# X1X1010/XequiNet

Hardware: AMD Instinct MI355X
Metric: edges/sec + achieved HBM GB/s, energy+force inference, QM9-shape batch (higher is better)
Workload: dtype f32

## Files before the change

include/xeq.h:

```cpp
#ifndef XEQ_H
#define XEQ_H
#include <stdint.h>

#ifdef __cplusplus
extern "C" {
#endif

enum { XEQ_F32 = 0, XEQ_F64 = 1 };
enum { XEQ_RBF_BESSEL = 0, XEQ_RBF_GAUSSIAN = 1, XEQ_RBF_EXPBERN = 2, XEQ_RBF_EXPNORM = 3 };
enum { XEQ_CUTOFF_COSINE = 0, XEQ_CUTOFF_POLYNOMIAL = 1 };
enum {
  XEQ_OK = 0,
  XEQ_ERR_INVALID_ARGUMENT = 1,
  XEQ_ERR_LAUNCH = 2,
  XEQ_ERR_UNSUPPORTED = 3
};

int xeq_version(void);
const char* xeq_last_error(void);
int64_t xeq_launch_count(void);
int64_t xeq_launch_names(int64_t first, char* buf, int64_t cap);


int xeq_csr_rowptr(const int64_t* keys, int64_t n_keys, int64_t n_rows, int32_t* rowptr, void* stream);
// ... 173 lines not shown
int xeq_message_param_grad_mc(int64_t n_nodes, int64_t n_edges, const int64_t* center, const int64_t* nbr, const void* tab, const void* h,
                              const void* xhat, const void* grad_s, const void* grad_x, int rbf_kind, int num_basis, int node_dim,
                              const int32_t mul[3], int xhat_layout, int grad_x_layout, const int32_t* n_valid, int n_parts, void* parts,
                              void* stream);
int xeq_norm_param_grad_chunks(int64_t n_nodes);
int xeq_norm_param_grad(const void* s, const void* x, const void* stats, const void* g_shat, int64_t ld_gs, const void* g_xhat_bt,
                        int64_t n_nodes, int node_dim, const int32_t mul[3], int n_chunks, void* parts, void* stream);
int xeq_to_bt(const void* x, int64_t n_nodes, const int32_t mul[3], void* out, void* stream);

int xeq_train_norm(int dtype, int reverse, int64_t n, const void* s, const void* s_tan, const void* x, const void* x_tan, const void* ln_w,
                   const void* ln_b, const void* eq_w, const void* eq_b, const void* g_s, const void* g_x, int node_dim,
                   const int32_t mul[3], double eps_ln, double eps_eq, int xhat_layout, void* out_s, void* out_x, void* rows, void* stream);
int xeq_train_uv(int dtype, int reverse, int64_t n, const void* const uv[3], const void* const uv_tan[3], const void* g, const int32_t mul[3],
                 double eps, void* out, void* const d_uv[3], void* stream);
int xeq_train_out(int dtype, int reverse, int64_t n, const void* const uv[3], const void* const uv_tan[3], const void* a, const void* a_tan,
                  const void* inner, const void* inner_tan, const void* g_s, const void* g_x, int node_dim, const int32_t mul[3],
                  void* out0, void* out1, void* const d_uv[3], void* stream);

#define XEQ_FAMILY_WQ 0
#define XEQ_FAMILY_SB 1
#define XEQ_FAMILY_GENERIC 3
int xeq_message_auto_family(int dtype, int64_t n_nodes, int64_t n_edges, int num_basis, int node_dim, const int32_t mul[3]);
int xeq_message_wq_edges_per_stream(int64_t n_nodes, int64_t n_edges);

int xeq_edge_basis_width(int num_basis);
int xeq_message_sb_fits(int64_t n_nodes, int64_t n_edges, int num_basis, int node_dim, const int32_t mul[3]);
int xeq_edge_basis(int dtype, const void* vec, int64_t n_edges, int rbf_kind, int cutoff_kind, int num_basis,
                   double cutoff, const void* p0, const void* p1, void* basis, void* dbasis, void* stream);
int xeq_message_fwd_sb(int dtype, int64_t n_nodes, int64_t n_edges, const int32_t* rowptr, const int32_t* perm,
                       const int64_t* nbr, const void* basis, const void* h, const void* xhat, const void* s_in,
                       const void* x_in, const void* w_rbf, const void* b_rbf, int num_basis, int node_dim,
                       const int32_t mul[3], void* s_out, void* x_out, int xhat_layout, void* stream);
int xeq_message_bwd_sb(int dtype, int64_t n_nodes, int64_t n_edges, const int32_t* n_rowptr, const int32_t* n_perm,
                       const int64_t* center, const void* basis, const void* dbasis, const void* h, const void* xhat,
                       const void* grad_s, const void* grad_x, const void* w_rbf, const void* b_rbf, int num_basis,
                       int node_dim, const int32_t mul[3], void* grad_h, void* grad_xhat, void* grad_vec,
                       int xhat_layout, void* stream);

#define XEQ_SB_Y0_ZERO 8
#define XEQ_SB_ACCUM_VEC 16
#define XEQ_SB_Q_ACCUMULATE 16
#define XEQ_SB_NO_GY 32
int xeq_message_bwd_sbq(int dtype, int64_t n_nodes, int64_t n_edges, const int32_t* n_rowptr, const int32_t* n_perm,
                        const int64_t* center, const void* basis, const void* h, const void* xhat, const void* grad_s,
                        const void* grad_x, const void* w_rbf, const void* b_rbf, int num_basis, int node_dim,
                        const int32_t mul[3], void* grad_h, void* grad_xhat, void* q, void* gy, int flags, void* stream);
int xeq_message_fwd_sb_pair(int dtype, int64_t n_nodes, int64_t n_edges, const int32_t* rowptr, const int32_t* perm, const int64_t* nbr,
                            const void* basis, const void* basis_u, const void* h, const void* u_h, const void* xhat, const void* u_xhat,
                            const void* s_in, const void* x_in, const void* w_rbf, const void* b_rbf, int num_basis, int node_dim,
                            const int32_t mul[3], void* s_out, void* x_out, int xhat_layout, void* stream);
int xeq_message_bwd_sbq_pair(int dtype, int64_t n_nodes, int64_t n_edges, const int32_t* n_rowptr, const int32_t* n_perm,
                             const int64_t* center, const void* basis, const void* basis_u, const void* h, const void* u_h, const void* xhat,
                             const void* u_xhat, const void* grad_s, const void* grad_x, const void* w_rbf, const void* b_rbf, int num_basis,
                             int node_dim, const int32_t mul[3], void* grad_h, void* grad_xhat, void* q, void* gy, int flags, void* stream);
int xeq_zero_rows_from(void* buf, int64_t row_words, int64_t n_rows, const int32_t* n_valid, void* stream);
int xeq_message_q_wgrad_chunks(int64_t n_edges);
int xeq_message_q_wgrad(int dtype, const void* q, const void* basis, int64_t n_edges, int num_basis, int node_dim, const int32_t mul[3],
                        int n_chunks, void* parts, void* stream);

int xeq_message_wq_supported(int num_basis, int node_dim, const int32_t mul[3]);
int xeq_message_wq_fits(int64_t n_nodes, int64_t n_edges, int num_basis, int node_dim, const int32_t mul[3]);
int64_t xeq_message_wq_pcap(int64_t n_nodes, int64_t n_edges);
int xeq_message_wq_waves(void);
int xeq_message_wq_record_floats_for(int num_basis);
int xeq_message_wq_record_floats(void);
int64_t xeq_message_wq_plan_workspace(int64_t n_nodes);
int64_t xeq_message_wq_win_ints(int n_ranges);
int xeq_message_wq_plan(const int32_t* rowptr, const int32_t* perm, const int64_t* owner, const int64_t* gather,
                        int64_t n_nodes, int64_t n_edges, int n_ranges, void* workspace, int64_t workspace_bytes,
                        int32_t* qptr, int32_t* pgath, int32_t* peid, int32_t* qinfo, int32_t* sq, int32_t* sn, int32_t* win,
                        void* stream);
int xeq_edge_basis_wq(const void* vec, int64_t n_nodes, int64_t n_edges, const int32_t* qptr, const int32_t* peid,
                      int rbf_kind, int cutoff_kind, int num_basis, double cutoff, const void* p0, const void* p1,
                      void* basis, void* dbasis, void* stream);
int xeq_message_fwd_wq(int64_t n_nodes, int64_t n_edges, int n_ranges, const int32_t* sq, const int32_t* sn, const int32_t* win,
                       const int32_t* c_rowptr, const int32_t* pgath, const int32_t* qinfo, const void* basis, const void* h,
                       const void* xhat, const void* s_in, const void* x_in, const void* w_rbf, const void* b_rbf,
                       int num_basis, int node_dim, const int32_t mul[3], void* s_out, void* x_out, int xhat_layout,
                       void* stream);
int64_t xeq_message_wq_parts_floats(int64_t n_nodes, int64_t n_edges, const int32_t mul[3]);
#define XEQ_XHAT_HIGHER_L_ZERO 2
#define XEQ_WQ_MIRROR_WALK 4
#define XEQ_WQ_PACKED_WEIGHTS 64
int64_t xeq_message_wq_packed_weight_floats(int num_basis, int node_dim, const int32_t mul[3]);
int xeq_message_wq_pack_weights(const void* w_rbf, const void* b_rbf, int num_basis, int node_dim, const int32_t mul[3], void* packed,
                                void* stream);
int xeq_message_bwd_wq(int64_t n_nodes, int64_t n_edges, int n_ranges, const int32_t* sq, const int32_t* sn, const int32_t* win,
                       const int32_t* n_rowptr, const int32_t* pgath, const int32_t* qinfo, const void* basis,
                       const void* dbasis, const void* h, const void* xhat, const void* grad_s, const void* grad_x,
                       const void* w_rbf, const void* b_rbf, int num_basis, int node_dim, const int32_t mul[3], void* grad_h,
                       void* grad_xhat, void* parts, int xhat_layout, void* stream);
int xeq_message_wq_edge_grad(const void* vec, int64_t n_nodes, int64_t n_edges, const int32_t* qptr, const int32_t* peid,
                             const int32_t* mirror, const int32_t mul[3], const void* parts, void* grad_vec, void* stream);
#define XEQ_WQ_MAX_PART_SETS 8
// ... 85 lines not shown
```

xequinet_amd/csrc/xeq_message_wq.hip:

```cpp
#include "xeq_common.h"

#include <hipcub/hipcub.hpp>
#include <stdlib.h>

namespace xeq {

typedef float f32x16 __attribute__((ext_vector_type(16)));
typedef float f32x4 __attribute__((ext_vector_type(4)));
typedef int i32x4 __attribute__((ext_vector_type(4)));

typedef __bf16 bf16x8 __attribute__((ext_vector_type(8)));

constexpr bool wq_bftail(int ks) { return ks <= 3; }
constexpr int WQ_TAIL = 24;
constexpr int wq_tailw(int ks) { return ks <= 4 ? 4 : 8; }
constexpr int wq_recf(int ks) { return WQ_TAIL + 2 * wq_tailw(ks) + 8; }
constexpr int wq_yoff(int ks) { return WQ_TAIL + 2 * wq_tailw(ks); }
constexpr int wq_tail_values(int num_basis) { return (num_basis > 16 ? num_basis - 16 : 0) + 1; }
constexpr int wq_ks(int num_basis) {
  return wq_tail_values(num_basis) <= 1 ? 1 : (wq_tail_values(num_basis) <= 5 ? 3 : ((wq_tail_values(num_basis) + 1) / 2 < 4 ? 4 : (wq_tail_values(num_basis) + 1) / 2));
}
constexpr int WQ_REC_MAX = 48;
__device__ __forceinline__ uint32_t wq_bf16_rne(float x) {
  const uint32_t u = __float_as_uint(x);
// ... 67 lines not shown
    qinfo[q0 + g] = (uint32_t)n | (g == 0 ? WQ_FIRST : 0u) | (g == nq - 1 ? WQ_LAST : 0u);
  }
}

__global__ void k_wq_streams(const int32_t* __restrict__ qptr, int64_t N, int n_ranges, int32_t* __restrict__ sq,
                             int32_t* __restrict__ sn) {
  const int k = blockIdx.x * blockDim.x + threadIdx.x;
  if (k > 2 * n_ranges) return;
  const int64_t Q = qptr[N];
  if (k == 2 * n_ranges) {
    sq[k] = (int32_t)Q;
    sn[k] = (int32_t)N;
    return;
  }
  const int64_t target = (int64_t)k * Q / (2 * n_ranges);
  int64_t lo = 0, hi = N;
  while (lo < hi) {
    const int64_t mid = (lo + hi) >> 1;
    if (qptr[mid] >= target) hi = mid;
    else lo = mid + 1;
  }
  sq[k] = qptr[lo];
  sn[k] = (int32_t)lo;
}

__global__ void k_wq_windows(const int32_t* __restrict__ sq, const int32_t* __restrict__ pgath, int n_ranges, int n_steps, int mult,
                             int32_t* __restrict__ win) {
  const int step = blockIdx.x, lane = threadIdx.x;
  if (step >= n_steps) return;
  const int k0 = min(2 * WQ_WAVES * mult * step, 2 * n_ranges), k1 = min(k0 + 2 * WQ_WAVES * mult, 2 * n_ranges);
  const int64_t p0 = 4 * (int64_t)sq[k0], p1 = 4 * (int64_t)sq[k1];
  int lo = 0x7fffffff, hi = -1;
  for (int64_t p = p0 + lane; p < p1; p += 64) {
    const int g = pgath[p];
    lo = g < lo ? g : lo;
    hi = g > hi ? g : hi;
  }
#pragma unroll
  for (int o = 32; o > 0; o >>= 1) {
    const int l2 = __shfl_xor(lo, o, 64), h2 = __shfl_xor(hi, o, 64);
    lo = l2 < lo ? l2 : lo;
    hi = h2 > hi ? h2 : hi;
  }
  if (lane == 0) {
    win[2 * step] = hi >= 0 ? lo : 0;
    win[2 * step + 1] = hi >= 0 ? hi - lo + 1 : 0;
// ... 1499 lines not shown
int xeq_message_wq_supported(int num_basis, int node_dim, const int32_t mul[3]) { return wq_supported(num_basis, node_dim, mul) ? 1 : 0; }

int xeq_message_wq_fits(int64_t n_nodes, int64_t n_edges, int num_basis, int node_dim, const int32_t mul[3]) {
  return wq_supported(num_basis, node_dim, mul) && n_nodes < (1ll << 30) && wq_fits(n_nodes, n_edges, node_dim, mul) ? 1 : 0;
}

int64_t xeq_message_wq_pcap(int64_t n_nodes, int64_t n_edges) { return wq_pcap(n_nodes, n_edges); }

int xeq_message_wq_waves(void) { return WQ_WAVES; }

int xeq_message_wq_record_floats(void) { return wq_recf(4); }
int xeq_message_wq_record_floats_for(int num_basis) { return wq_recf(wq_ks(num_basis)); }

int64_t xeq_message_wq_plan_workspace(int64_t n_nodes) {
  size_t temp = 0;
  QuadCount op{nullptr, n_nodes};
  hipcub::CountingInputIterator<int64_t> cnt(0);
  hipcub::TransformInputIterator<int32_t, QuadCount, hipcub::CountingInputIterator<int64_t>> it(cnt, op);
  if (hipcub::DeviceScan::ExclusiveSum(nullptr, temp, it, (int32_t*)nullptr, (int)(n_nodes + 1)) != hipSuccess) return -1;
  return (int64_t)temp + 256;
}

int xeq_message_wq_plan(const int32_t* rowptr, const int32_t* perm, const int64_t* owner, const int64_t* gather,
                        int64_t n_nodes, int64_t n_edges, int n_ranges, void* workspace, int64_t workspace_bytes,
                        int32_t* qptr, int32_t* pgath, int32_t* peid, int32_t* qinfo, int32_t* sq, int32_t* sn, int32_t* win,
                        void* stream) {
  XEQ_CHECK_ARG(n_nodes >= 0 && n_edges >= 0 && n_ranges >= 1 && n_nodes < (1ll << 30) && n_edges < (1ll << 31), "xeq_message_wq_plan: bad sizes");
  const int64_t need = xeq_message_wq_plan_workspace(n_nodes);
  XEQ_CHECK_ARG(need >= 0 && workspace_bytes >= need, "xeq_message_wq_plan: workspace of %lld bytes, need %lld", (long long)workspace_bytes, (long long)need);
  QuadCount op{rowptr, n_nodes};
  if (n_nodes <= SCAN_WG_MAX_ITEMS) {
    static const bool attr_ok = hipFuncSetAttribute((const void*)k_wq_quad_scan, hipFuncAttributeMaxDynamicSharedMemorySize,
                                                    (int)wg_scan_lds_bytes(SCAN_WG_MAX_ITEMS)) == hipSuccess;
    XEQ_CHECK_ARG(attr_ok, "xeq_message_wq_plan: cannot reserve LDS for the quad scan");
    hipLaunchKernelGGL(k_wq_quad_scan, dim3(1), dim3(SCAN_WG_THREADS), wg_scan_lds_bytes(n_nodes), (hipStream_t)stream, op, qptr);
    XEQ_CHECK_LAUNCH("xeq_message_wq_plan (quad scan)");
  } else {
    hipcub::CountingInputIterator<int64_t> cnt(0);
    hipcub::TransformInputIterator<int32_t, QuadCount, hipcub::CountingInputIterator<int64_t>> it(cnt, op);
    size_t temp = (size_t)workspace_bytes;
    if (hipcub::DeviceScan::ExclusiveSum(workspace, temp, it, qptr, (int)(n_nodes + 1), (hipStream_t)stream) != hipSuccess) {
      xeq::set_error("xeq_message_wq_plan: scan failed");
      return XEQ_ERR_LAUNCH;
    }
  }
  if (n_edges + n_nodes > 0) {
    hipLaunchKernelGGL(k_wq_fill, dim3((unsigned)((n_edges + n_nodes + 255) / 256)), dim3(256), 0, (hipStream_t)stream, n_edges, n_nodes,
                       rowptr, perm, owner, gather, (const int32_t*)qptr, pgath, peid, (uint32_t*)qinfo);
    XEQ_CHECK_LAUNCH("xeq_message_wq_plan (fill)");
  }
  const int n = 2 * n_ranges + 1;
  hipLaunchKernelGGL(k_wq_streams, dim3((unsigned)((n + 255) / 256)), dim3(256), 0, (hipStream_t)stream, (const int32_t*)qptr,
                     n_nodes, n_ranges, sq, sn);
  XEQ_CHECK_LAUNCH("xeq_message_wq_plan (streams)");
  const int n_steps = wq_class_steps(n_ranges, 1);
  hipLaunchKernelGGL(k_wq_windows, dim3((unsigned)n_steps), dim3(64), 0, (hipStream_t)stream, (const int32_t*)sq,
                     (const int32_t*)pgath, n_ranges, n_steps, 1, win);
  XEQ_CHECK_LAUNCH("xeq_message_wq_plan (windows)");
  const int mlong = wq_long_mult(n_edges, n_ranges);
  if (mlong > 1) {
    const int n_long = wq_class_steps(n_ranges, mlong);
    hipLaunchKernelGGL(k_wq_windows, dim3((unsigned)n_long), dim3(64), 0, (hipStream_t)stream, (const int32_t*)sq,
                       (const int32_t*)pgath, n_ranges, n_long, mlong, win + 2 * n_steps);
    XEQ_CHECK_LAUNCH("xeq_message_wq_plan (windows, long class)");
  }
  return XEQ_OK;
}

int64_t xeq_message_wq_win_ints(int n_ranges) {
  return 2 * ((int64_t)wq_class_steps(n_ranges, 1) + (int64_t)wq_class_steps(n_ranges, 2) + 1);
}

int xeq_edge_basis_wq(const void* vec, int64_t n_nodes, int64_t n_edges, const int32_t* qptr, const int32_t* peid,
                      int rbf_kind, int cutoff_kind, int num_basis, double cutoff, const void* p0, const void* p1,
                      void* basis, void* dbasis, void* stream) {
  XEQ_CHECK_ARG(n_edges >= 0 && n_nodes >= 0 && num_basis >= 1 && num_basis <= 31 && cutoff > 0, "xeq_edge_basis_wq: bad sizes");
  XEQ_CHECK_ARG(rbf_kind >= XEQ_RBF_BESSEL && rbf_kind <= XEQ_RBF_EXPNORM, "xeq_edge_basis_wq: rbf kernel %d is not implemented", rbf_kind);
  XEQ_CHECK_ARG(rbf_kind == XEQ_RBF_BESSEL || p1 != nullptr, "xeq_edge_basis_wq: this radial basis needs its second parameter array (std / logc / mu)");
  XEQ_CHECK_ARG(cutoff_kind == XEQ_CUTOFF_COSINE || cutoff_kind == XEQ_CUTOFF_POLYNOMIAL, "xeq_edge_basis_wq: cutoff function %d is not implemented", cutoff_kind);
  if (n_edges == 0 && n_nodes == 0) return XEQ_OK;
  const int64_t pcap = wq_pcap(n_nodes, n_edges), total = (pcap + WQ_REC_SLOTS - 1) / WQ_REC_SLOTS * 256;
  const int ks = wq_ks(num_basis);
  XEQ_CHECK_ARG(pcap * wq_recf(ks) < (1ll << 31) * 2, "xeq_edge_basis_wq: too many edges for 32-bit record offsets (shard the batch)");
  RadialSpec rs{rbf_kind, cutoff_kind, num_basis, cutoff};
  hipLaunchKernelGGL(k_wq_records, dim3((unsigned)((total + 255) / 256)), dim3(256), 0, (hipStream_t)stream, (const float*)vec,
                     peid, qptr, n_nodes, pcap, rs, (const float*)p0, (const float*)p1, (float*)basis, (float*)dbasis, wq_recf(ks), wq_tailw(ks), wq_bftail(ks) ? 1 : 0);
  XEQ_CHECK_LAUNCH("xeq_edge_basis_wq");
  return XEQ_OK;
}

// ... 154 lines not shown
```

xequinet_amd/csrc/xeq_ops.hip:

```cpp
#include "xeq_common.h"

namespace xeq {

template <typename T>
__global__ void k_edge_vectors_fwd(const T* __restrict__ pos, const int64_t* __restrict__ edge_index, int64_t E,
                                   const T* __restrict__ cell, const T* __restrict__ cell_offsets,
                                   const int64_t* __restrict__ batch, T* __restrict__ vec, T* __restrict__ dist) {
  int64_t e = (int64_t)blockIdx.x * blockDim.x + threadIdx.x;
  if (e >= E) return;
  int64_t c = edge_index[e], n = edge_index[E + e];
  T v[3];
#pragma unroll
  for (int a = 0; a < 3; ++a) v[a] = pos[3 * c + a] - pos[3 * n + a];
  if (cell != nullptr) {
    const T* cm = cell + (batch ? 9 * batch[n] : 0);
    T o0 = cell_offsets[3 * e], o1 = cell_offsets[3 * e + 1], o2 = cell_offsets[3 * e + 2];
#pragma unroll
    for (int a = 0; a < 3; ++a) v[a] -= o0 * cm[a] + o1 * cm[3 + a] + o2 * cm[6 + a];
  }
  vec[3 * e] = v[0];
  vec[3 * e + 1] = v[1];
  vec[3 * e + 2] = v[2];
  if (dist) dist[e] = sqrt_<T>(v[0] * v[0] + v[1] * v[1] + v[2] * v[2]);
}
// ... 303 lines not shown

__global__ void k_compare_many(CopyMany cm, int32_t gen, int32_t* __restrict__ flag) {
  const int b = blockIdx.y;
  const int64_t words = cm.bytes[b] / 4;
  const uint32_t* x = reinterpret_cast<const uint32_t*>(cm.src[b]);
  const uint32_t* y = reinterpret_cast<const uint32_t*>(cm.dst[b]);
  bool diff = false;
  for (int64_t i = (int64_t)blockIdx.x * blockDim.x + threadIdx.x; i < words; i += (int64_t)gridDim.x * blockDim.x) diff |= x[i] != y[i];
  if (__ballot(diff) != 0ull && (threadIdx.x & 63) == 0) flag[0] = gen;
}

}

using namespace xeq;

#define XEQ_IRREPS(who)                       \
  Irreps ir;                                  \
  {                                           \
    int rc_ = check_irreps(mul, ir, who);     \
    if (rc_ != XEQ_OK) return rc_;            \
  }

#include <atomic>
static std::atomic<long long> g_pack_epoch{0};

extern "C" {

long long xeq_pack_epoch(void) { return g_pack_epoch.load(); }
void xeq_pack_epoch_bump(void) { g_pack_epoch.fetch_add(1); }


int xeq_message_auto_family(int dtype, int64_t n_nodes, int64_t n_edges, int num_basis, int node_dim, const int32_t mul[3]) {
  const bool f32 = dtype == XEQ_F32;
  const bool sb_fits = xeq_message_sb_fits(n_nodes, n_edges, num_basis, node_dim, mul) != 0;
  if (n_edges < 4096 && sb_fits) return XEQ_FAMILY_SB;
  if (f32 && xeq_message_wq_fits(n_nodes, n_edges, num_basis, node_dim, mul)) return XEQ_FAMILY_WQ;
  if (sb_fits) return XEQ_FAMILY_SB;
  return XEQ_FAMILY_GENERIC;
}

int64_t xeq_small_rows_limit(void) { return xeq_small_rows(); }

int xeq_message_wq_edges_per_stream(int64_t n_nodes, int64_t n_edges) {
  const double per_node = (double)n_edges / (double)(n_nodes > 0 ? n_nodes : 1);
  double v = per_node > 16.0 ? per_node : 16.0;
  const double spread = (double)n_edges / 1500.0;
  if (spread > v) v = spread;
  if (v > 80.0) v = 80.0;
  return (int)v;
}


int xeq_edge_vectors_fwd(int dtype, const void* pos, const int64_t* edge_index, int64_t n_edges,
                         const void* cell, const void* cell_offsets, const int64_t* batch, void* vec, void* dist,
                         void* stream) {
  XEQ_CHECK_ARG(n_edges >= 0, "xeq_edge_vectors_fwd: n_edges < 0");
  XEQ_CHECK_ARG((cell == nullptr) == (cell_offsets == nullptr), "xeq_edge_vectors_fwd: cell and cell_offsets must both be given or both be NULL (data/transform.py:67-68)");
  if (n_edges == 0) return XEQ_OK;
  XEQ_DISPATCH_FLOAT(dtype, {
    hipLaunchKernelGGL((k_edge_vectors_fwd<T>), dim3((unsigned)((n_edges + 255) / 256)), dim3(256), 0,
                       (hipStream_t)stream, (const T*)pos, edge_index, n_edges, (const T*)cell,
                       (const T*)cell_offsets, batch, (T*)vec, (T*)dist);
  });
  XEQ_CHECK_LAUNCH("xeq_edge_vectors_fwd");
  return XEQ_OK;
}

int xeq_edge_vectors_bwd(int dtype, const void* grad_vec, int64_t n_nodes, const int32_t* c_rowptr,
                         const int32_t* c_perm, const int32_t* n_rowptr, const int32_t* n_perm, void* grad_pos,
                         void* stream) {
  XEQ_CHECK_ARG(n_nodes >= 0, "xeq_edge_vectors_bwd: n_nodes < 0");
  if (n_nodes == 0) return XEQ_OK;
// ... 289 lines not shown
```

xequinet_amd/csrc/xeq_torch.cpp:

```cpp
#include <ATen/ATen.h>
#include <c10/hip/HIPStream.h>
#include <hip/hip_runtime_api.h>
#include <torch/csrc/autograd/custom_function.h>
#include <torch/library.h>

#include <array>
#include <cmath>
#include <cstdlib>
#include <map>
#include <mutex>
#include <optional>
#include <unordered_map>
#include <vector>

#include "../../include/xeq.h"

namespace {

using at::Tensor;
using torch::autograd::AutogradContext;
using torch::autograd::variable_list;

#define XCALL(...)                                                                                  \
  do {                                                                                              \
// ... 225 lines not shown
struct NbPacks { Tensor fwd, bwd, bias_uv; };
const NbPacks* nb_packs(const Tensor* q, const Tensor* qn, bool gx) {
  const bool tail = qn != nullptr;
  const Tensor none;
  return &packed<NbPacks>(q[15].data_ptr(), {&q[15], &q[10], &q[11], &q[12], &q[14], &q[17], &q[13], tail ? &qn[0] : &none, tail ? &qn[2] : &none},
                          (tail ? 2 : 0) + (gx ? 1 : 0), [&](NbPacks& e) {
    const auto bopt = q[15].options().dtype(at::kByte);
    const Tensor w3 = q[15].detach().contiguous(), dot = q[14].detach().contiguous(), w4 = q[17].detach().contiguous();
    const Tensor uv0 = q[10].contiguous(), uv1 = q[11].contiguous(), uv2 = q[12].contiguous();
    Tensor w1n, w2n;
    if (tail) {
      w1n = qn[0].detach().contiguous();
      w2n = qn[2].detach().contiguous();
    }
    e.fwd = at::empty({xeq_node_block_fwd_tiles(tail) * 3072}, bopt);
    XCALL(xeq_node_block_pack_fwd(PF(w3), PF(uv0), PF(uv1), PF(uv2), PF(dot), PF(w4), PF(w1n), PF(w2n), e.fwd.data_ptr(), cur_stream()));
    e.bwd = at::empty({xeq_node_block_bwd_tiles(tail, gx) * 3072}, bopt);
    XCALL(xeq_node_block_pack_bwd(PF(w3), PF(uv0), PF(uv1), PF(uv2), PF(dot), PF(w4), PF(w1n), PF(w2n), gx, e.bwd.data_ptr(), cur_stream()));
    e.bias_uv = q[13].numel() > 0 ? q[13].detach().contiguous() : Tensor();
  });
}

struct WqPlan {
  int n_ranges = 0;
  int64_t pcap = 0;
  Tensor qptr, pgath, peid, qinfo, sq, sn, win, rowptr, work, basis, dbasis;
};
struct Graph {
  int64_t N = 0, E = 0;
  bool mirror = false;
  Tensor ei, c_rowptr, c_perm, n_rowptr, n_perm;
  Tensor mirror_map;
  WqPlan fwd, rev;
  Tensor sb_basis, sb_dbasis;
  void sorted_view();
  const Tensor& rev_rowptr() { if (!mirror_map.defined()) sorted_view(); return mirror_map.defined() ? c_rowptr : n_rowptr; }
  const Tensor& rev_perm() { if (!mirror_map.defined()) sorted_view(); return mirror_map.defined() ? mirror_map : n_perm; }
};

Tensor i32(int64_t n, const Tensor& like) { return at::empty({std::max<int64_t>(n, 1)}, like.options().dtype(at::kInt)); }

void csr_by_key(const Tensor& keys, int64_t n_rows, Tensor& rowptr, Tensor& perm) {
  const int64_t n = keys.numel(), bytes = xeq_csr_by_key_workspace(n, n_rows);
  TORCH_CHECK(bytes >= 0, "xequinet_amd: csr_by_key: sizes out of range");
  Tensor work = at::empty({std::max<int64_t>(bytes, 1)}, keys.options().dtype(at::kByte));
  rowptr = i32(n_rows + 1, keys);
  perm = i32(n, keys);
// ... 19 lines not shown
  }
  const char* env = std::getenv("XEQ_PBC_MIRROR");
  const bool periodic = cell_offsets != nullptr && cell_offsets->defined();
  g.mirror = symmetric && center_sorted && (!periodic || !(env && env[0] == '0' && env[1] == 0));
  if (g.mirror && !periodic) {
    g.n_rowptr = g.c_rowptr;
    g.n_perm = i32(g.E, g.ei);
    XCALL(xeq_reverse_edge_map((const int64_t*)g.ei.data_ptr(), g.E, n_nodes, (const int32_t*)g.c_rowptr.data_ptr(),
                               (int32_t*)g.n_perm.data_ptr(), cur_stream()));
    g.mirror_map = g.n_perm;
  } else if (g.mirror) {
    g.mirror_map = i32(g.E, g.ei);
    XCALL(xeq_reverse_edge_map_pbc(dcode(*cell_offsets), (const int64_t*)g.ei.data_ptr(), cell_offsets->data_ptr(), g.E, n_nodes,
                                   (const int32_t*)g.c_rowptr.data_ptr(), (int32_t*)g.mirror_map.data_ptr(), cur_stream()));
  } else {
    g.sorted_view();
  }
  return g;
}

void build_wq_plan(Graph& g, bool reverse, WqPlan& p) {
  if (reverse) g.sorted_view();
  const int eps = xeq_message_wq_edges_per_stream(g.N, g.E);
  p.n_ranges = (int)std::max<int64_t>(1, (g.E + 2 * eps - 1) / (2 * eps));
  p.pcap = xeq_message_wq_pcap(g.N, g.E);
  p.qptr = i32(g.N + 1, g.ei);
  p.pgath = i32(p.pcap, g.ei);
  p.peid = i32(p.pcap, g.ei);
  p.qinfo = i32(p.pcap / 4, g.ei);
  p.sq = i32(2 * p.n_ranges + 1, g.ei);
  p.sn = i32(2 * p.n_ranges + 1, g.ei);
  p.win = i32(xeq_message_wq_win_ints(p.n_ranges), g.ei);
  const int64_t wbytes = xeq_message_wq_plan_workspace(g.N);
  TORCH_CHECK(wbytes >= 0, "xequinet_amd: wq plan workspace");
  p.work = at::empty({std::max<int64_t>(wbytes, 1)}, g.ei.options().dtype(at::kByte));
  p.rowptr = reverse ? g.n_rowptr : g.c_rowptr;
  const Tensor& perm = reverse ? g.n_perm : g.c_perm;
  const Tensor owner = g.ei.select(0, reverse ? 1 : 0), gather = g.ei.select(0, reverse ? 0 : 1);
  XCALL(xeq_message_wq_plan((const int32_t*)p.rowptr.data_ptr(), perm.defined() ? (const int32_t*)perm.data_ptr() : nullptr,
                            (const int64_t*)owner.data_ptr(), (const int64_t*)gather.data_ptr(), g.N, g.E, p.n_ranges,
                            p.work.data_ptr(), wbytes, (int32_t*)p.qptr.data_ptr(), (int32_t*)p.pgath.data_ptr(),
                            (int32_t*)p.peid.data_ptr(), (int32_t*)p.qinfo.data_ptr(), (int32_t*)p.sq.data_ptr(),
                            (int32_t*)p.sn.data_ptr(), (int32_t*)p.win.data_ptr(), cur_stream()));
}

constexpr int P_BLOCK0 = 5, P_PER_BLOCK = 27, P_ELECTRONIC = 6;
struct Hyper {
  int F, mul[3], B, blocks, rbf_kind, cutoff_kind, layer_norm, embed_kind;
  double cutoff, inv_eps;
  int C() const { return mul[0] + mul[1] + mul[2]; }
  int D() const { return mul[0] + 3 * mul[1] + 5 * mul[2]; }
  int H() const { return F + 2 * C(); }
};

const Tensor* opt(const Tensor& t) { return t.defined() && t.numel() > 0 ? &t : nullptr; }
const void* OP(const Tensor& t) { return t.defined() && t.numel() > 0 ? t.data_ptr() : nullptr; }

struct BtBlock {
  int l, m;
  Tensor view;
};
std::vector<BtBlock> bt_blocks(const Tensor& buf, int64_t n, const int mul[3], int width) {
  std::vector<BtBlock> out;
  int64_t base = 0;
// ... 737 lines not shown
```

xequinet_amd/lib.py:

```python
from __future__ import annotations

import ctypes
import os
from ctypes import c_char_p, c_double, c_int, c_int32, c_int64, c_void_p
from typing import Optional

import torch

_HERE = os.path.dirname(os.path.abspath(__file__))
LIB_PATH = os.environ.get("XEQ_LIB_PATH") or os.path.join(_HERE, "libxeq_hip.so")

XEQ_F32, XEQ_F64 = 0, 1
COPY_MANY_MAX = 16
SB_ACCUM_VEC = 16
XHAT_HIGHER_L_ZERO = 2
SB_Y0_ZERO = 8
SB_Q_ACCUMULATE = 16
SB_NO_GY = 32
WQ_MIRROR_WALK = 4
WQ_PACKED_WEIGHTS = 64
WQ_MAX_PART_SETS = 8
RBF_KINDS = {"bessel": 0, "gaussian": 1, "expbern": 2, "expnorm": 3}
CUTOFF_KINDS = {"cosine": 0, "polynomial": 1}

# ... 88 lines not shown
    "xeq_edge_basis_width": [c_int],
    "xeq_edge_basis": [c_int, _P, c_int64, c_int, c_int, c_int, c_double, _P, _P, _P, _P, _P],
    "xeq_message_fwd_sb": [c_int, c_int64, c_int64, _P, _P, _P, _P, _P, _P, _P, _P, _P, _P, c_int, c_int, _I3, _P, _P, c_int, _P],
    "xeq_message_bwd_sbq": [c_int, c_int64, c_int64, _P, _P, _P, _P, _P, _P, _P, _P, _P, _P, c_int, c_int, _I3, _P, _P, _P, _P, c_int, _P],
    "xeq_message_q_wgrad": [c_int, _P, _P, c_int64, c_int, c_int, _I3, c_int, _P, _P],
    "xeq_message_q_wgrad_chunks": [c_int64],
    "xeq_train_norm": [c_int, c_int, c_int64, _P, _P, _P, _P, _P, _P, _P, _P, _P, _P, c_int, _I3, c_double, c_double, c_int, _P, _P, _P, _P],
    "xeq_train_uv": [c_int, c_int, c_int64, _P, _P, _P, _I3, c_double, _P, _P, _P],
    "xeq_train_out": [c_int, c_int, c_int64, _P, _P, _P, _P, _P, _P, _P, _P, c_int, _I3, _P, _P, _P, _P],
    "xeq_zero_rows_from": [_P, c_int64, c_int64, _P, _P],
    "xeq_message_fwd_sb_pair": [c_int, c_int64, c_int64, _P, _P, _P, _P, _P, _P, _P, _P, _P, _P, _P, _P, _P, c_int, c_int, _I3, _P, _P, c_int, _P],
    "xeq_message_bwd_sbq_pair": [c_int, c_int64, c_int64, _P, _P, _P, _P, _P, _P, _P, _P, _P, _P, _P, _P, _P, c_int, c_int, _I3, _P, _P, _P, _P, c_int, _P],
    "xeq_message_bwd_sb": [c_int, c_int64, c_int64, _P, _P, _P, _P, _P, _P, _P, _P, _P, _P, _P, c_int, c_int, _I3, _P, _P, _P,
                           c_int, _P],
    "xeq_message_sb_fits": [c_int64, c_int64, c_int, c_int, _I3],
    "xeq_message_wq_supported": [c_int, c_int, _I3],
    "xeq_message_wq_fits": [c_int64, c_int64, c_int, c_int, _I3],
    "xeq_message_wq_pcap": [c_int64, c_int64],
    "xeq_message_wq_waves": [],
    "xeq_message_wq_record_floats": [],
    "xeq_message_wq_record_floats_for": [c_int],
    "xeq_message_wq_plan_workspace": [c_int64],
    "xeq_message_wq_win_ints": [c_int],
    "xeq_message_wq_plan": [_P, _P, _P, _P, c_int64, c_int64, c_int, _P, c_int64, _P, _P, _P, _P, _P, _P, _P, _P],
    "xeq_edge_basis_wq": [_P, c_int64, c_int64, _P, _P, c_int, c_int, c_int, c_double, _P, _P, _P, _P, _P],
    "xeq_message_fwd_wq": [c_int64, c_int64, c_int, _P, _P, _P, _P, _P, _P, _P, _P, _P, _P, _P, _P, _P, c_int, c_int, _I3,
                           _P, _P, c_int, _P],
    "xeq_message_wq_parts_floats": [c_int64, c_int64, _I3],
    "xeq_message_bwd_wq": [c_int64, c_int64, c_int, _P, _P, _P, _P, _P, _P, _P, _P, _P, _P, _P, _P, _P, _P, c_int, c_int,
                           _I3, _P, _P, _P, c_int, _P],
    "xeq_message_wq_packed_weight_floats": [c_int, c_int, _I3],
    "xeq_message_wq_pack_weights": [_P, _P, c_int, c_int, _I3, _P, _P],
    "xeq_message_wq_edge_grad": [_P, c_int64, c_int64, _P, _P, _P, _I3, _P, _P, _P],
    "xeq_message_wq_edge_grad_sum": [_P, c_int64, c_int64, _P, _P, _P, _I3, c_int, ctypes.POINTER(c_void_p), _P, _P],
    "xeq_norm_fwd": [c_int, _P, _P, _P, _P, _P, _P, c_int64, c_int, _I3, c_int, _P, c_int64, _P, _P, _P],
    "xeq_norm_bwd": [c_int, _P, _P, _P, _P, _P, c_int64, c_int, _I3, c_int, _P, c_int64, _P, _P, _P, _P, _P, _P],
    "xeq_uv_reduce_fwd": [c_int, _P, c_int64, _I3, c_double, _P, c_int64, c_int, _P, _P],
    "xeq_uv_reduce_bwd": [c_int, _P, _P, _P, c_int64, c_int, c_int64, _I3, c_double, _P, _P, _P, _P],
    "xeq_update_out_fwd": [c_int, _P, _P, _P, _P, _P, c_int64, c_int, _I3, _P, _P, _P],
    "xeq_update_out_bwd": [c_int, _P, _P, _P, _P, _P, c_int64, c_int, _I3, _P, _P, _P, _P],
    "xeq_update_uv_supported": [c_int, c_int, _I3],
    "xeq_update_uv_fwd": [_P, _P, _P, _P, _P, _P, c_int64, c_int, _I3, c_int, _P, _P, _P, c_int, c_double, _P, c_int64, _P, _P, _P, _P],
    "xeq_update_uv_bwd": [_P, _P, _P, c_int64, _P, _P, _P, c_int64, _P, _P, _P, _P, _P, c_int64, c_int, _I3, c_int, _P, _P, _P, c_double,
                          _P, _P, _P, _P],
    "xeq_mlp2_supported": [c_int, c_int, c_int, c_int],
    "xeq_node_tile_split": [c_int64, c_int, ctypes.POINTER(c_int64)],
    "xeq_mlp_packed_floats": [c_int, c_int],
    "xeq_mlp_pack": [_P, _P, c_int, c_int, c_int, _P, _P],
    "xeq_mlp2_fwd": [_P, c_int64, c_int64, c_int, _P, _P, c_int, _P, _P, c_int64, _P],
    "xeq_mlp2_bwd": [_P, c_int64, c_int64, c_int, _P, _P, _P, c_int, _P, c_int64, _P],
    "xeq_mlp2_and_linear": [c_int, _P, c_int64, c_int64, c_int, _P, _P, c_int, _P, _P, c_int64, _P, c_int64, c_int, _P, c_int, _P, c_int64, _P],
    "xeq_pack_epoch": [],
    "xeq_pack_epoch_bump": [],
    "xeq_rowptr_guard": [_P, c_int64, c_int64, _P, _P, _P],
    "xeq_node_block_supported": [c_int, c_int, _I3],
    "xeq_node_block_fwd_tiles": [c_int],
    "xeq_node_block_rows": [c_int64],
    "xeq_node_block_auto": [c_int64],
    "xeq_small_rows_limit": [],
    "xeq_node_block_set_waves": [c_int],
    "xeq_node_block_pack_fwd": [_P, _P, _P, _P, _P, _P, _P, _P, _P, _P],
    "xeq_node_block_fwd": [c_int64, _P, _P, _P, _P, _P, _P, _P, _P, _P, c_double, _P, _P, _P, _P, _P, _P, _P, _P, _P, _P, _P, _P, _P, _P, _P,
                           _P, _P, _P, _P, _P],
    "xeq_node_block_linear_test": [_P, c_int64, _P, c_int, c_int, _P, _P, _P],
    "xeq_node_block_bwd_tiles": [c_int, c_int],
    "xeq_node_block_pack_bwd": [_P, _P, _P, _P, _P, _P, _P, _P, c_int, _P, _P],
    "xeq_node_block_bwd": [c_int64, _P, _P, _P, _P, _P, _P, _P, _P, _P, _P, _P, _P, _P, _P, _P, _P, _P, _P, _P, c_double, _P, _P, _P, _P, _P,
                           _P, _P, _P],
}
_RET_I64 = {"xeq_launch_count", "xeq_launch_names", "xeq_message_wq_packed_weight_floats", "xeq_rowptr_from_degrees_max", "xeq_csr_by_key_workspace", "xeq_message_wq_pcap", "xeq_message_wq_plan_workspace", "xeq_message_wq_win_ints",
            "xeq_message_wq_parts_floats", "xeq_mlp_packed_floats", "xeq_exclusive_scan_i32_workspace", "xeq_node_block_fwd_tiles", "xeq_node_block_bwd_tiles", "xeq_node_block_rows", "xeq_pack_epoch", "xeq_tensor_product_wgrad_chunks", "xeq_small_rows_limit"}
EXPORTS = ["xeq_version", "xeq_last_error", *_PROTOS]

_lib: Optional[ctypes.CDLL] = None


def load() -> ctypes.CDLL:
    global _lib
    if _lib is not None:
        return _lib
    if not os.path.exists(LIB_PATH):
        raise ImportError(
            f"{LIB_PATH} not found: build it with `python -m xequinet_amd.csrc.build` "
            "(xequinet_amd has no CPU / pure-PyTorch fallback)"
        )
    lib = ctypes.CDLL(LIB_PATH)
    lib.xeq_version.restype = c_int
    lib.xeq_last_error.restype = c_char_p
    for name, argtypes in _PROTOS.items():
        fn = getattr(lib, name)
        fn.argtypes = argtypes
        fn.restype = c_int64 if name in _RET_I64 else c_int
    _lib = lib
# ... 81 lines not shown
```

xequinet_amd/ops.py:

```python
from __future__ import annotations

import ctypes
from typing import Optional, Tuple

import torch
from torch.autograd import Function
from torch.autograd.function import once_differentiable

from . import lib
from .lib import call, dtype_code, mul3, ptr, require_hip, stream


class _KernelTimer:

    def __init__(self) -> None:
        self.enabled = False
        self.events = {}

    def reset(self, enabled: bool) -> None:
        self.enabled = enabled
        self.events = {}

    def launch(self, name: str, *args, label: Optional[str] = None) -> None:
        if not self.enabled:
# ... 132 lines not shown

    @property
    def n_rowptr(self) -> torch.Tensor:
        return self._sorted_neighbor_view()[0]

    @property
    def n_perm(self) -> torch.Tensor:
        return self._sorted_neighbor_view()[1]

    def reverse_view(self):
        if self.mirror_map is not None:
            return self.c_rowptr, self.mirror_map
        return self._sorted_neighbor_view()

    def wq_plan(self, reverse: bool, edges_per_stream: int = 128):
        key = (bool(reverse), int(edges_per_stream))
        if self._wq is None:
            self._wq = {}
        plan = self._wq.get(key)
        if plan is None:
            L = lib.load()
            N, E, dev = self.n_nodes, self.n_edges, self.edge_index.device
            pcap = int(L.xeq_message_wq_pcap(N, E))
            n_ranges = max(1, -(-E // (2 * edges_per_stream)))
            i32 = lambda n: torch.empty(max(int(n), 1), dtype=torch.int32, device=dev)
            plan = {"reverse": bool(reverse), "n_ranges": n_ranges, "pcap": pcap, "qptr": i32(N + 1), "pgath": i32(pcap),
                    "peid": i32(pcap), "qinfo": i32(pcap // 4), "sq": i32(2 * n_ranges + 1), "sn": i32(2 * n_ranges + 1),
                    "win": i32(int(L.xeq_message_wq_win_ints(n_ranges))),
                    "work": torch.empty(max(int(L.xeq_message_wq_plan_workspace(N)), 1), dtype=torch.uint8, device=dev),
                    "records": None}
            self._wq[key] = plan
            self._build_wq_plan(plan)
        return plan

    def _build_wq_plan(self, plan) -> None:
        rev = plan["reverse"]
        rowptr, perm = (self.n_rowptr, self.n_perm) if rev else (self.c_rowptr, self.c_perm)
        owner, gather = (self.edge_index[1], self.edge_index[0]) if rev else (self.edge_index[0], self.edge_index[1])
        plan["rowptr"] = rowptr
        call("xeq_message_wq_plan", ptr(rowptr), ptr(perm), ptr(owner), ptr(gather), self.n_nodes, self.n_edges, plan["n_ranges"],
             ptr(plan["work"]), plan["work"].numel(), ptr(plan["qptr"]), ptr(plan["pgath"]), ptr(plan["peid"]), ptr(plan["qinfo"]),
             ptr(plan["sq"]), ptr(plan["sn"]), ptr(plan["win"]), stream())

    def refresh_plans(self) -> None:
        for plan in (self._wq or {}).values():
            self._build_wq_plan(plan)



_CELL_LIST_MIN_ATOMS = 512
_CELL_LIST_MAX_BINS = 64


def _use_cell_list(n_atoms: int, n_graphs: int) -> bool:
    import os

    flag = os.environ.get("XEQ_CELL_LIST")
    if flag is not None:
        return flag not in ("0", "", "false")
    return n_atoms >= _CELL_LIST_MIN_ATOMS * max(1, n_graphs)


def _radius_graph_cell_list(pos, ptr_, cutoff):
    N, G = pos.shape[0], ptr_.numel() - 1
# ... 924 lines not shown
```

Baseline: 177.4 million.

## Pack WQ message streams per step by tile capacity instead of equal quad splits

Adds a step-aware stream planner. Quads are cut into per-step node ranges, and a ballot search finds the smallest tile capacity that packs each step's 2*WAVES streams. The change also alters how many ranges get allocated. The goal is to balance work across the waves of each step so the longest stream shrinks and idle waves are reduced in the message kernels. The cost is a more complex planning kernel and possibly more ranges and steps. An env var can fall back to the old equal split.

```diff
diff --git a/include/xeq.h b/include/xeq.h
--- a/include/xeq.h
+++ b/include/xeq.h
@@ -219,6 +219,8 @@
 #define XEQ_FAMILY_GENERIC 3
 int xeq_message_auto_family(int dtype, int64_t n_nodes, int64_t n_edges, int num_basis, int node_dim, const int32_t mul[3]);
 int xeq_message_wq_edges_per_stream(int64_t n_nodes, int64_t n_edges);
+int xeq_message_wq_tiles_per_stream(int64_t n_nodes, int64_t n_edges, int edges_per_stream);
+int xeq_message_wq_plan_ranges(int64_t n_nodes, int64_t n_edges, int edges_per_stream, int tiles);
 
 int xeq_edge_basis_width(int num_basis);
 int xeq_message_sb_fits(int64_t n_nodes, int64_t n_edges, int num_basis, int node_dim, const int32_t mul[3]);
@@ -264,9 +266,12 @@
 int64_t xeq_message_wq_plan_workspace(int64_t n_nodes);
 int64_t xeq_message_wq_win_ints(int n_ranges);
 int xeq_message_wq_plan(const int32_t* rowptr, const int32_t* perm, const int64_t* owner, const int64_t* gather,
-                        int64_t n_nodes, int64_t n_edges, int n_ranges, void* workspace, int64_t workspace_bytes,
+                        int64_t n_nodes, int64_t n_edges, int n_ranges, int tiles, void* workspace, int64_t workspace_bytes,
                         int32_t* qptr, int32_t* pgath, int32_t* peid, int32_t* qinfo, int32_t* sq, int32_t* sn, int32_t* win,
                         void* stream);
+int xeq_message_wq_plan_host(const int32_t* rowptr, int64_t n_nodes, int n_ranges, int tiles, int32_t* qptr, int32_t* sq, int32_t* sn,
+                             int32_t* step_tiles);
+int64_t xeq_message_wq_step_quads(int64_t n_quads, int64_t n_nodes, int tiles);
 int xeq_edge_basis_wq(const void* vec, int64_t n_nodes, int64_t n_edges, const int32_t* qptr, const int32_t* peid,
                       int rbf_kind, int cutoff_kind, int num_basis, double cutoff, const void* p0, const void* p1,
                       void* basis, void* dbasis, void* stream);
diff --git a/xequinet_amd/csrc/xeq_message_wq.hip b/xequinet_amd/csrc/xeq_message_wq.hip
--- a/xequinet_amd/csrc/xeq_message_wq.hip
+++ b/xequinet_amd/csrc/xeq_message_wq.hip
@@ -113,6 +113,101 @@
   }
   sq[k] = qptr[lo];
   sn[k] = (int32_t)lo;
+}
+
+__host__ __device__ __forceinline__ int64_t wq_step_quads(int64_t Q, int64_t N, int tiles) {
+  const int64_t cap = 2 * WQ_WAVES * 4 * (int64_t)tiles;
+  const int64_t x = cap - (N > 0 ? (2 * WQ_WAVES * 11 * Q) / (20 * N) : 0);
+  return x < cap / 2 ? cap / 2 : x;
+}
+__host__ __device__ __forceinline__ int wq_steps_used(int64_t Q, int64_t N, int tiles, int n_table) {
+  const int64_t x = wq_step_quads(Q, N, tiles), u = (Q + x - 1) / x;
+  return (int)(u < 1 ? 1 : (u > n_table ? n_table : u));
+}
+__host__ __device__ __forceinline__ int64_t wq_step_cut(const int32_t* __restrict__ qptr, int64_t N, int64_t Q, int u, int n_used) {
+  if (u >= n_used) return N;
+  const int64_t target = (int64_t)u * Q / n_used;
+  int64_t lo = 0, hi = N;
+  while (lo < hi) {
+    const int64_t mid = (lo + hi) >> 1;
+    if (qptr[mid] >= target) hi = mid;
+    else lo = mid + 1;
+  }
+  return lo;
+}
+__host__ __device__ __forceinline__ int wq_step_index(int s, int n_used, int n_table) { return (int)((int64_t)s * n_used / n_table); }
+template <typename QP>
+__host__ __device__ __forceinline__ bool wq_pack_step(QP qp, int cnt, int ns, int cap, int bounds[2 * WQ_WAVES + 1]) {
+  int start = 0;
+  bounds[0] = 0;
+#pragma unroll
+  for (int j = 0; j < 2 * WQ_WAVES; ++j) {
+    if (j < ns) {
+      const int64_t limit = (int64_t)qp(start) + cap;
+      int lo = start, hi = cnt;
+      while (lo < hi) {
+        const int mid = (lo + hi + 1) >> 1;
+        if (qp(mid) <= limit) lo = mid;
+        else hi = mid - 1;
+      }
+      start = lo;
+    }
+    bounds[j + 1] = start;
+  }
+  return start == cnt;
+}
+__host__ __device__ __forceinline__ int wq_step_min_tiles(int64_t quads, int ns) {
+  const int64_t t = (quads + 4 * ns - 1) / (4 * ns);
+  return (int)(t < 1 ? 1 : t);
+}
+
+constexpr int WQ_PLAN_LDS_NODES = 1024;
+__global__ void __launch_bounds__(64) k_wq_step_streams(const int32_t* __restrict__ qptr, int64_t N, int n_ranges, int tiles,
+                                                        int32_t* __restrict__ sq, int32_t* __restrict__ sn) {
+  __shared__ int32_t q_l[WQ_PLAN_LDS_NODES + 1];
+  const int s = blockIdx.x, lane = threadIdx.x, K = 2 * n_ranges, n_table = (n_ranges + WQ_WAVES - 1) / WQ_WAVES;
+  if (s >= n_table) return;
+  const int64_t Q = qptr[N];
+  const int n_used = wq_steps_used(Q, N, tiles, n_table);
+  const int u0 = wq_step_index(s, n_used, n_table), u1 = wq_step_index(s + 1, n_used, n_table);
+  const int k0 = 2 * WQ_WAVES * s, ns = min(2 * WQ_WAVES, K - k0);
+  const int mine = (int)wq_step_cut(qptr, N, Q, lane == 0 ? u0 : u1, n_used);
+  const int a = __shfl(mine, 0, 64), b = __shfl(mine, 1, 64), cnt = b - a;
+  if (s == n_table - 1 && lane == 0) {
+    sq[K] = (int32_t)Q;
+    sn[K] = (int32_t)N;
+  }
+  if (cnt <= 0) {
+    if (lane < ns) {
+      sq[k0 + lane] = qptr[a];
+      sn[k0 + lane] = a;
+    }
+    return;
+  }
+  const bool in_lds = cnt <= WQ_PLAN_LDS_NODES;
+  if (in_lds) {
+    for (int i = lane; i <= cnt; i += 64) q_l[i] = qptr[a + i];
+    __syncthreads();
+  }
+  const int q_a = qptr[a], quads = qptr[b] - q_a;
+  int bounds[2 * WQ_WAVES + 1];
+  for (int t0 = wq_step_min_tiles(quads, ns);; t0 += 64) {
+    const int cap = 4 * (t0 + lane);
+    const bool ok = in_lds ? wq_pack_step([&](int i) { return q_l[i]; }, cnt, ns, cap, bounds)
+                           : wq_pack_step([&](int i) { return qptr[a + i]; }, cnt, ns, cap, bounds);
+    const unsigned long long fits = __ballot(ok);
+    if (fits) {
+      if (lane == __ffsll((long long)fits) - 1) {
+#pragma unroll
+        for (int j = 0; j < 2 * WQ_WAVES; ++j)
+          if (j < ns) {
+            sq[k0 + j] = in_lds ? q_l[bounds[j]] : qptr[a + bounds[j]];
+            sn[k0 + j] = a + bounds[j];
+          }
+      }
+      return;
+    }
+  }
 }
 
 __global__ void k_wq_windows(const int32_t* __restrict__ sq, const int32_t* __restrict__ pgath, int n_ranges, int n_steps, int mult,
@@ -1658,10 +1753,11 @@
 }
 
 int xeq_message_wq_plan(const int32_t* rowptr, const int32_t* perm, const int64_t* owner, const int64_t* gather,
-                        int64_t n_nodes, int64_t n_edges, int n_ranges, void* workspace, int64_t workspace_bytes,
+                        int64_t n_nodes, int64_t n_edges, int n_ranges, int tiles, void* workspace, int64_t workspace_bytes,
                         int32_t* qptr, int32_t* pgath, int32_t* peid, int32_t* qinfo, int32_t* sq, int32_t* sn, int32_t* win,
                         void* stream) {
   XEQ_CHECK_ARG(n_nodes >= 0 && n_edges >= 0 && n_ranges >= 1 && n_nodes < (1ll << 30) && n_edges < (1ll << 31), "xeq_message_wq_plan: bad sizes");
+  XEQ_CHECK_ARG(tiles <= 4096, "xeq_message_wq_plan: %d tiles per stream", tiles);
   const int64_t need = xeq_message_wq_plan_workspace(n_nodes);
   XEQ_CHECK_ARG(need >= 0 && workspace_bytes >= need, "xeq_message_wq_plan: workspace of %lld bytes, need %lld", (long long)workspace_bytes, (long long)need);
   QuadCount op{rowptr, n_nodes};
@@ -1686,10 +1782,14 @@
     XEQ_CHECK_LAUNCH("xeq_message_wq_plan (fill)");
   }
   const int n = 2 * n_ranges + 1;
-  hipLaunchKernelGGL(k_wq_streams, dim3((unsigned)((n + 255) / 256)), dim3(256), 0, (hipStream_t)stream, (const int32_t*)qptr,
-                     n_nodes, n_ranges, sq, sn);
+  const int n_steps = wq_class_steps(n_ranges, 1);
+  if (tiles > 0)
+    hipLaunchKernelGGL(k_wq_step_streams, dim3((unsigned)n_steps), dim3(64), 0, (hipStream_t)stream, (const int32_t*)qptr, n_nodes,
+                       n_ranges, tiles, sq, sn);
+  else
+    hipLaunchKernelGGL(k_wq_streams, dim3((unsigned)((n + 255) / 256)), dim3(256), 0, (hipStream_t)stream, (const int32_t*)qptr,
+                       n_nodes, n_ranges, sq, sn);
   XEQ_CHECK_LAUNCH("xeq_message_wq_plan (streams)");
-  const int n_steps = wq_class_steps(n_ranges, 1);
   hipLaunchKernelGGL(k_wq_windows, dim3((unsigned)n_steps), dim3(64), 0, (hipStream_t)stream, (const int32_t*)sq,
                      (const int32_t*)pgath, n_ranges, n_steps, 1, win);
   XEQ_CHECK_LAUNCH("xeq_message_wq_plan (windows)");
@@ -1702,6 +1802,63 @@
   }
   return XEQ_OK;
 }
+
+int xeq_message_wq_plan_host(const int32_t* rowptr, int64_t n_nodes, int n_ranges, int tiles, int32_t* qptr, int32_t* sq, int32_t* sn,
+                             int32_t* step_tiles) {
+  XEQ_CHECK_ARG(rowptr && qptr && sq && sn && n_nodes >= 0 && n_ranges >= 1 && n_nodes < (1ll << 30) && tiles <= 4096, "xeq_message_wq_plan_host: bad arguments");
+  const QuadCount op{rowptr, n_nodes};
+  int64_t run = 0;
+  for (int64_t i = 0; i < n_nodes; ++i) {
+    qptr[i] = (int32_t)run;
+    run += op(i);
+  }
+  XEQ_CHECK_ARG(run < (1ll << 31), "xeq_message_wq_plan_host: too many quads");
+  qptr[n_nodes] = (int32_t)run;
+  const int64_t N = n_nodes, Q = run;
+  const int K = 2 * n_ranges, n_table = (n_ranges + WQ_WAVES - 1) / WQ_WAVES;
+  sq[K] = (int32_t)Q;
+  sn[K] = (int32_t)N;
+  if (tiles <= 0) {
+    for (int k = 0; k < K; ++k) {
+      const int64_t target = (int64_t)k * Q / K;
+      int64_t lo = 0, hi = N;
+      while (lo < hi) {
+        const int64_t mid = (lo + hi) >> 1;
+        if (qptr[mid] >= target) hi = mid;
+        else lo = mid + 1;
+      }
+      sq[k] = qptr[lo];
+      sn[k] = (int32_t)lo;
+    }
+  } else {
+    const int n_used = wq_steps_used(Q, N, tiles, n_table);
+    for (int s = 0; s < n_table; ++s) {
+      const int k0 = 2 * WQ_WAVES * s, ns = K - k0 < 2 * WQ_WAVES ? K - k0 : 2 * WQ_WAVES;
+      const int a = (int)wq_step_cut(qptr, N, Q, wq_step_index(s, n_used, n_table), n_used);
+      const int b = (int)wq_step_cut(qptr, N, Q, wq_step_index(s + 1, n_used, n_table), n_used);
+      const int cnt = b - a;
+      int bounds[2 * WQ_WAVES + 1] = {0};
+      if (cnt > 0) {
+        const int32_t* q = qptr + a;
+        for (int t = wq_step_min_tiles(qptr[b] - qptr[a], ns);; ++t)
+          if (wq_pack_step([&](int i) { return q[i]; }, cnt, ns, 4 * t, bounds)) break;
+      }
+      for (int j = 0; j < ns; ++j) {
+        sq[k0 + j] = qptr[a + bounds[j]];
+        sn[k0 + j] = a + bounds[j];
+      }
+    }
+  }
+  if (step_tiles)
+    for (int s = 0; s < n_table; ++s) {
+      int longest = 0;
+      for (int k = 2 * WQ_WAVES * s; k < 2 * WQ_WAVES * (s + 1) && k < K; ++k) longest = sq[k + 1] - sq[k] > longest ? sq[k + 1] - sq[k] : longest;
+      step_tiles[s] = (longest + 3) >> 2;
+    }
+  return XEQ_OK;
+}
+
+int64_t xeq_message_wq_step_quads(int64_t n_quads, int64_t n_nodes, int tiles) { return wq_step_quads(n_quads, n_nodes, tiles < 1 ? 1 : tiles); }
 
 int64_t xeq_message_wq_win_ints(int n_ranges) {
   return 2 * ((int64_t)wq_class_steps(n_ranges, 1) + (int64_t)wq_class_steps(n_ranges, 2) + 1);
diff --git a/xequinet_amd/csrc/xeq_ops.hip b/xequinet_amd/csrc/xeq_ops.hip
--- a/xequinet_amd/csrc/xeq_ops.hip
+++ b/xequinet_amd/csrc/xeq_ops.hip
@@ -349,6 +349,8 @@
   }
 
 #include <atomic>
+#include <stdlib.h>
+#include <string.h>
 static std::atomic<long long> g_pack_epoch{0};
 
 extern "C" {
@@ -375,6 +377,34 @@
   if (spread > v) v = spread;
   if (v > 80.0) v = 80.0;
   return (int)v;
+}
+
+int xeq_message_wq_tiles_per_stream(int64_t n_nodes, int64_t n_edges, int edges_per_stream) {
+  const char* mode = getenv("XEQ_WQ_PLAN");
+  if (mode && strcmp(mode, "equal") == 0) return 0;
+  const int eps = edges_per_stream > 0 ? edges_per_stream : xeq_message_wq_edges_per_stream(n_nodes, n_edges);
+  int base = 8;
+  const char* env = getenv("XEQ_WQ_TILES");
+  if (env && atoi(env) >= 1 && atoi(env) <= 16) base = atoi(env);
+  int64_t t = ((int64_t)eps * base + 79) / 80;
+  t = t < 1 ? 1 : (t > 4096 ? 4096 : t);
+  const int64_t q_est = n_edges / 4 + (3 * n_nodes + 7) / 8 + 1;
+  if (q_est > t * (n_nodes > 0 ? n_nodes : 1)) return 0;
+  return (int)t;
+}
+
+int xeq_message_wq_plan_ranges(int64_t n_nodes, int64_t n_edges, int edges_per_stream, int tiles) {
+  const int64_t cap = (1ll << 30);
+  if (tiles <= 0) {
+    const int64_t eps = edges_per_stream > 0 ? edges_per_stream : 1;
+    const int64_t r = (n_edges + 2 * eps - 1) / (2 * eps);
+    return (int)(r < 1 ? 1 : (r > cap ? cap : r));
+  }
+  const int64_t q_est = n_edges / 4 + (3 * n_nodes + 7) / 8 + 1;
+  const int64_t x = xeq_message_wq_step_quads(q_est, n_nodes, tiles);
+  const int64_t steps = (q_est + q_est / 32 + x - 1) / x + 1;
+  const int64_t r = steps * xeq_message_wq_waves();
+  return (int)(r > cap ? cap : r);
 }
 
 
diff --git a/xequinet_amd/csrc/xeq_torch.cpp b/xequinet_amd/csrc/xeq_torch.cpp
--- a/xequinet_amd/csrc/xeq_torch.cpp
+++ b/xequinet_amd/csrc/xeq_torch.cpp
@@ -271,7 +271,7 @@
 }
 
 struct WqPlan {
-  int n_ranges = 0;
+  int n_ranges = 0, tiles = 0;
   int64_t pcap = 0;
   Tensor qptr, pgath, peid, qinfo, sq, sn, win, rowptr, work, basis, dbasis;
 };
@@ -337,7 +337,8 @@
 void build_wq_plan(Graph& g, bool reverse, WqPlan& p) {
   if (reverse) g.sorted_view();
   const int eps = xeq_message_wq_edges_per_stream(g.N, g.E);
-  p.n_ranges = (int)std::max<int64_t>(1, (g.E + 2 * eps - 1) / (2 * eps));
+  p.tiles = xeq_message_wq_tiles_per_stream(g.N, g.E, eps);
+  p.n_ranges = xeq_message_wq_plan_ranges(g.N, g.E, eps, p.tiles);
   p.pcap = xeq_message_wq_pcap(g.N, g.E);
   p.qptr = i32(g.N + 1, g.ei);
   p.pgath = i32(p.pcap, g.ei);
@@ -354,7 +355,7 @@
   const Tensor owner = g.ei.select(0, reverse ? 1 : 0), gather = g.ei.select(0, reverse ? 0 : 1);
   XCALL(xeq_message_wq_plan((const int32_t*)p.rowptr.data_ptr(), perm.defined() ? (const int32_t*)perm.data_ptr() : nullptr,
                             (const int64_t*)owner.data_ptr(), (const int64_t*)gather.data_ptr(), g.N, g.E, p.n_ranges,
-                            p.work.data_ptr(), wbytes, (int32_t*)p.qptr.data_ptr(), (int32_t*)p.pgath.data_ptr(),
+                            p.tiles, p.work.data_ptr(), wbytes, (int32_t*)p.qptr.data_ptr(), (int32_t*)p.pgath.data_ptr(),
                             (int32_t*)p.peid.data_ptr(), (int32_t*)p.qinfo.data_ptr(), (int32_t*)p.sq.data_ptr(),
                             (int32_t*)p.sn.data_ptr(), (int32_t*)p.win.data_ptr(), cur_stream()));
 }
diff --git a/xequinet_amd/lib.py b/xequinet_amd/lib.py
--- a/xequinet_amd/lib.py
+++ b/xequinet_amd/lib.py
@@ -134,7 +134,11 @@
     "xeq_message_wq_record_floats_for": [c_int],
     "xeq_message_wq_plan_workspace": [c_int64],
     "xeq_message_wq_win_ints": [c_int],
-    "xeq_message_wq_plan": [_P, _P, _P, _P, c_int64, c_int64, c_int, _P, c_int64, _P, _P, _P, _P, _P, _P, _P, _P],
+    "xeq_message_wq_plan": [_P, _P, _P, _P, c_int64, c_int64, c_int, c_int, _P, c_int64, _P, _P, _P, _P, _P, _P, _P, _P],
+    "xeq_message_wq_plan_host": [_P, c_int64, c_int, c_int, _P, _P, _P, _P],
+    "xeq_message_wq_step_quads": [c_int64, c_int64, c_int],
+    "xeq_message_wq_tiles_per_stream": [c_int64, c_int64, c_int],
+    "xeq_message_wq_plan_ranges": [c_int64, c_int64, c_int, c_int],
     "xeq_edge_basis_wq": [_P, c_int64, c_int64, _P, _P, c_int, c_int, c_int, c_double, _P, _P, _P, _P, _P],
     "xeq_message_fwd_wq": [c_int64, c_int64, c_int, _P, _P, _P, _P, _P, _P, _P, _P, _P, _P, _P, _P, _P, c_int, c_int, _I3,
                            _P, _P, c_int, _P],
@@ -180,7 +184,7 @@
     "xeq_node_block_bwd": [c_int64, _P, _P, _P, _P, _P, _P, _P, _P, _P, _P, _P, _P, _P, _P, _P, _P, _P, _P, _P, c_double, _P, _P, _P, _P, _P,
                            _P, _P, _P],
 }
-_RET_I64 = {"xeq_launch_count", "xeq_launch_names", "xeq_message_wq_packed_weight_floats", "xeq_rowptr_from_degrees_max", "xeq_csr_by_key_workspace", "xeq_message_wq_pcap", "xeq_message_wq_plan_workspace", "xeq_message_wq_win_ints",
+_RET_I64 = {"xeq_launch_count", "xeq_launch_names", "xeq_message_wq_packed_weight_floats", "xeq_rowptr_from_degrees_max", "xeq_csr_by_key_workspace", "xeq_message_wq_pcap", "xeq_message_wq_plan_workspace", "xeq_message_wq_win_ints", "xeq_message_wq_step_quads",
             "xeq_message_wq_parts_floats", "xeq_mlp_packed_floats", "xeq_exclusive_scan_i32_workspace", "xeq_node_block_fwd_tiles", "xeq_node_block_bwd_tiles", "xeq_node_block_rows", "xeq_pack_epoch", "xeq_tensor_product_wgrad_chunks", "xeq_small_rows_limit"}
 EXPORTS = ["xeq_version", "xeq_last_error", *_PROTOS]
 
diff --git a/xequinet_amd/ops.py b/xequinet_amd/ops.py
--- a/xequinet_amd/ops.py
+++ b/xequinet_amd/ops.py
@@ -178,9 +178,10 @@
             L = lib.load()
             N, E, dev = self.n_nodes, self.n_edges, self.edge_index.device
             pcap = int(L.xeq_message_wq_pcap(N, E))
-            n_ranges = max(1, -(-E // (2 * edges_per_stream)))
+            tiles = int(L.xeq_message_wq_tiles_per_stream(N, E, int(edges_per_stream)))
+            n_ranges = int(L.xeq_message_wq_plan_ranges(N, E, int(edges_per_stream), tiles))
             i32 = lambda n: torch.empty(max(int(n), 1), dtype=torch.int32, device=dev)
-            plan = {"reverse": bool(reverse), "n_ranges": n_ranges, "pcap": pcap, "qptr": i32(N + 1), "pgath": i32(pcap),
+            plan = {"reverse": bool(reverse), "n_ranges": n_ranges, "tiles": tiles, "pcap": pcap, "qptr": i32(N + 1), "pgath": i32(pcap),
                     "peid": i32(pcap), "qinfo": i32(pcap // 4), "sq": i32(2 * n_ranges + 1), "sn": i32(2 * n_ranges + 1),
                     "win": i32(int(L.xeq_message_wq_win_ints(n_ranges))),
                     "work": torch.empty(max(int(L.xeq_message_wq_plan_workspace(N)), 1), dtype=torch.uint8, device=dev),
@@ -195,7 +196,7 @@
         owner, gather = (self.edge_index[1], self.edge_index[0]) if rev else (self.edge_index[0], self.edge_index[1])
         plan["rowptr"] = rowptr
         call("xeq_message_wq_plan", ptr(rowptr), ptr(perm), ptr(owner), ptr(gather), self.n_nodes, self.n_edges, plan["n_ranges"],
-             ptr(plan["work"]), plan["work"].numel(), ptr(plan["qptr"]), ptr(plan["pgath"]), ptr(plan["peid"]), ptr(plan["qinfo"]),
+             plan["tiles"], ptr(plan["work"]), plan["work"].numel(), ptr(plan["qptr"]), ptr(plan["pgath"]), ptr(plan["peid"]), ptr(plan["qinfo"]),
              ptr(plan["sq"]), ptr(plan["sn"]), ptr(plan["win"]), stream())
 
     def refresh_plans(self) -> None:
```

Result: no change. 177.6 million, median of 3 (+0.1%).
